# nanoporetech/bonito

Hardware: AMD Instinct MI355X
Metric: signal samples/sec/GPU (chunk=10000, batch=512) + read accuracy vs ref (higher is better)
Workload: dtype f16

## Files before the change

bonito_amd/csrc/conv.hip:

```cpp
#include "common.h"
#include "kernels.h"
#include "options.h"
#include <cstring>

namespace bh {

struct ConvFirstArgs {
    const half_t* sig;
    const float* w;
    const float* bias;
    half_t* out;
    int N, Lin, Lout, Cout, K, stride, pad, act;
    float clamp_lo, clamp_hi;
    long os_n, os_t;
    int vec8;
};

__global__ __launch_bounds__(256) void conv_first_kernel(ConvFirstArgs p) {
    extern __shared__ __attribute__((aligned(16))) char smem[];
    float* wl = (float*)smem;
    float* bl = wl + p.Cout * p.K;
    float* sl = bl + p.Cout;
    const int n = blockIdx.y;
    const int tb = blockIdx.x * 256;
    const int span = 255 * p.stride + p.K;
    const half_t* s = p.sig + (long)n * p.Lin;
    for (int i = threadIdx.x; i < p.Cout * p.K; i += 256) wl[i] = p.w[i];
    for (int i = threadIdx.x; i < p.Cout; i += 256) bl[i] = p.bias ? p.bias[i] : 0.0f;
    for (int i = threadIdx.x; i < span; i += 256) {
        int pos = tb * p.stride - p.pad + i;
        sl[i] = (pos >= 0 && pos < p.Lin) ? (float)s[pos] : 0.0f;
    }
    __syncthreads();
    const int t = tb + threadIdx.x;
    if (t >= p.Lout) return;
    const float* x = sl + threadIdx.x * p.stride;
    half_t* dst = p.out + (long)n * p.os_n + (long)t * p.os_t;
    auto channel = [&](int c) {
        const float* wr = wl + c * p.K;
        float a = bl[c];
        for (int k = 0; k < p.K; ++k) a = fmaf(wr[k], x[k], a);
        a = apply_act_rt(a, p.act);
        return (half_t)fminf(fmaxf(a, p.clamp_lo), p.clamp_hi);
    };
    int c0 = 0;
    if (p.vec8) {
        if (p.K == 5 && p.act == ACT_SWISH) {
            const float x0 = x[0], x1 = x[1], x2 = x[2], x3 = x[3], x4 = x[4];
            for (; c0 + 8 <= p.Cout; c0 += 8) {
                half8_t o;
#pragma unroll
                for (int j = 0; j < 8; ++j) {
                    const float* wr = wl + (c0 + j) * 5;
                    float a = bl[c0 + j];
                    a = fmaf(wr[0], x0, a);
                    a = fmaf(wr[1], x1, a);
                    a = fmaf(wr[2], x2, a);
                    a = fmaf(wr[3], x3, a);
                    a = fmaf(wr[4], x4, a);
                    o[j] = (half_t)fminf(fmaxf(swishf_(a), p.clamp_lo), p.clamp_hi);
                }
                *(half8_t*)(dst + c0) = o;
            }
        }
        for (; c0 + 8 <= p.Cout; c0 += 8) {
            half8_t o;
#pragma unroll
            for (int j = 0; j < 8; ++j) o[j] = channel(c0 + j);
            *(half8_t*)(dst + c0) = o;
        }
    }
    for (; c0 < p.Cout; ++c0) dst[c0] = channel(c0);
}

struct ConvArgs {
    const half_t* in;
    const half_t* wpk;
    const float* bias;
    half_t* out;
    int N, Lin, Lout, Cin, Cout, K, stride, pad, act;
    int Kp;
    float clamp_lo, clamp_hi;
    long os_n, os_t;
};

template <int NTT, bool FS = false>
__global__ __launch_bounds__(256) void conv_igemm_kernel(ConvArgs p) {
    extern __shared__ __attribute__((aligned(16))) char smem[];
    half_t* xin = (half_t*)smem;
    constexpr int PW = NTT * 16;
    constexpr int PB = 4 * PW;
    const int tid = threadIdx.x, lane = tid & 63, wave = tid >> 6;
    const int r = lane & 15, kg = lane >> 4;
    const int n = blockIdx.y;
    const int t0 = blockIdx.x * PB;

    const int span_pos = (PB - 1) * p.stride + p.K;
    const int span_halves = span_pos * p.Cin + 32 + 8;
    const int p_start = t0 * p.stride - p.pad;
    const half_t* src = p.in + (long)n * p.Lin * p.Cin;
    for (int e = tid * 8; e < span_halves; e += 256 * 8) {
        int pos = p_start + e / p.Cin;
        uint4_t v = {0, 0, 0, 0};
        if (pos >= 0 && pos < p.Lin && e < span_pos * p.Cin)
            v = *(const uint4_t*)(src + (long)pos * p.Cin + (e % p.Cin));
        *(uint4_t*)(xin + e) = v;
    }
    __syncthreads();

    const int nks = p.Kp >> 5;
    const int nft = (p.Cout + 15) >> 4;
    constexpr int NT = FS ? 4 * NTT : NTT;
    const int pbase = FS ? 0 : wave * PW;
    int boff[NT];
#pragma unroll
    for (int tt = 0; tt < NT; ++tt)
        boff[tt] = (pbase + tt * 16 + r) * p.stride * p.Cin + kg * 8;

    for (int ft = FS ? wave : 0; ft < nft; ft += FS ? 4 : 1) {
        float4_t acc[NT];
#pragma unroll
        for (int tt = 0; tt < NT; ++tt) acc[tt] = float4_t{0.f, 0.f, 0.f, 0.f};
        const half_t* wrow = p.wpk + (long)(ft * 16 + r) * p.Kp + kg * 8;
        int ks = 0;
        for (; FS && ks + 4 <= nks; ks += 4) {
            half8_t a[4];
#pragma unroll
            for (int u = 0; u < 4; ++u) a[u] = *(const half8_t*)(wrow + (ks + u) * 32);
#pragma unroll
            for (int u = 0; u < 4; ++u)
#pragma unroll
                for (int tt = 0; tt < NT; ++tt) {
                    half8_t b = *(const half8_t*)(xin + boff[tt] + (ks + u) * 32);
                    acc[tt] = mfma16(a[u], b, acc[tt]);
                }
        }
        for (; ks < nks; ++ks) {
            half8_t a = *(const half8_t*)(wrow + ks * 32);
#pragma unroll
            for (int tt = 0; tt < NT; ++tt) {
                half8_t b = *(const half8_t*)(xin + boff[tt] + ks * 32);
                acc[tt] = mfma16(a, b, acc[tt]);
            }
        }
        const int f = ft * 16 + kg * 4;
        if (f < p.Cout) {
            float bv[4];
#pragma unroll
            for (int g = 0; g < 4; ++g) bv[g] = (p.bias && f + g < p.Cout) ? p.bias[f + g] : 0.0f;
#pragma unroll
            for (int tt = 0; tt < NT; ++tt) {
                int t = t0 + pbase + tt * 16 + r;
                if (t >= p.Lout) continue;
                float xv[4];
#pragma unroll
                for (int g = 0; g < 4; ++g) xv[g] = acc[tt][g] + bv[g];
                if (p.act == ACT_SWISH) {
#pragma unroll
                    for (int g = 0; g < 4; ++g) xv[g] = swishf_(xv[g]);
                } else {
#pragma unroll
                    for (int g = 0; g < 4; ++g) xv[g] = apply_act_rt(xv[g], p.act);
                }
                half4_t o;
#pragma unroll
                for (int g = 0; g < 4; ++g) o[g] = (half_t)fminf(fmaxf(xv[g], p.clamp_lo), p.clamp_hi);
                half_t* dst = p.out + (long)n * p.os_n + (long)t * p.os_t + f;
                if (f + 4 <= p.Cout) *(half4_t*)dst = o;
                else
                    for (int g = 0; g < 4; ++g)
                        if (f + g < p.Cout) dst[g] = o[g];
            }
        }
    }
}

template <int FPW, int NKS, int WAVES>
__global__ __launch_bounds__(64 * WAVES) void conv_ws_kernel(ConvArgs p) {
    extern __shared__ __attribute__((aligned(16))) char smem[];
    half_t* xin = (half_t*)smem;
    constexpr int PB = 256;
    const int tid = threadIdx.x, lane = tid & 63, wave = tid >> 6;
    const int r = lane & 15, kg = lane >> 4;
    const int n = blockIdx.y;
    const int t0 = blockIdx.x * PB;

    half8_t afr[FPW][NKS];
#pragma unroll
    for (int f = 0; f < FPW; ++f) {
        const half_t* wrow = p.wpk + (long)((wave * FPW + f) * 16 + r) * p.Kp + kg * 8;
#pragma unroll
        for (int ks = 0; ks < NKS; ++ks) afr[f][ks] = *(const half8_t*)(wrow + ks * 32);
    }
    float4_t bv[FPW];
#pragma unroll
    for (int f = 0; f < FPW; ++f) {
        bv[f] = float4_t{0.f, 0.f, 0.f, 0.f};
        if (p.bias) bv[f] = *(const float4_t*)(p.bias + (wave * FPW + f) * 16 + kg * 4);
    }

    const int span_pos = (PB - 1) * p.stride + p.K;
    const int span_halves = span_pos * p.Cin + 32 + 8;
    const int p_start = t0 * p.stride - p.pad;
    const half_t* src = p.in + (long)n * p.Lin * p.Cin;
    for (int e = tid * 8; e < span_halves; e += 64 * WAVES * 8) {
        int pos = p_start + e / p.Cin;
        uint4_t v = {0, 0, 0, 0};
        if (pos >= 0 && pos < p.Lin && e < span_pos * p.Cin)
            v = *(const uint4_t*)(src + (long)pos * p.Cin + (e % p.Cin));
        *(uint4_t*)(xin + e) = v;
    }
    __syncthreads();

    const int RS = p.stride * p.Cin;
    for (int pt = 0; pt < PB / 16; ++pt) {
        const int t = t0 + pt * 16 + r;
        if (t0 + pt * 16 >= p.Lout) break;
        const half_t* xrow = xin + (pt * 16 + r) * RS + kg * 8;
        half8_t b[NKS];
#pragma unroll
        for (int ks = 0; ks < NKS; ++ks) b[ks] = *(const half8_t*)(xrow + ks * 32);
        float4_t acc[FPW];
#pragma unroll
        for (int f = 0; f < FPW; ++f) acc[f] = float4_t{0.f, 0.f, 0.f, 0.f};
#pragma unroll
        for (int ks = 0; ks < NKS; ++ks)
#pragma unroll
            for (int f = 0; f < FPW; ++f) acc[f] = mfma16(afr[f][ks], b[ks], acc[f]);
#pragma unroll
        for (int f = 0; f < FPW; ++f)
#pragma unroll
            for (int g = 0; g < 4; ++g) acc[f][g] += bv[f][g];
        switch (p.act) {
            case ACT_SWISH:
#pragma unroll
                for (int f = 0; f < FPW; ++f)
#pragma unroll
                    for (int g = 0; g < 4; ++g) acc[f][g] = swishf_(acc[f][g]);
                break;
            case ACT_TANH:
#pragma unroll
                for (int f = 0; f < FPW; ++f)
#pragma unroll
                    for (int g = 0; g < 4; ++g) acc[f][g] = tanhf_(acc[f][g]);
                break;
            case ACT_RELU:
#pragma unroll
                for (int f = 0; f < FPW; ++f)
#pragma unroll
                    for (int g = 0; g < 4; ++g) acc[f][g] = fmaxf(acc[f][g], 0.0f);
                break;
            default: break;
        }
        if (t < p.Lout) {
            half_t* drow = p.out + (long)n * p.os_n + (long)t * p.os_t + kg * 4;
#pragma unroll
            for (int f = 0; f < FPW; ++f) {
                half4_t o;
#pragma unroll
                for (int g = 0; g < 4; ++g) o[g] = (half_t)fminf(fmaxf(acc[f][g], p.clamp_lo), p.clamp_hi);
                *(half4_t*)(drow + (wave * FPW + f) * 16) = o;
            }
        }
    }
}

struct ConvFront3Args {
    const half_t* sig;
    const float* w1;
    const float* b1;
    const half_t* w2pk;
    const float* b2;
    int L0, L1, L2;
    int K1, pad1, act1;
    int K2, pad2, act2;
    float lo1, hi1, lo2, hi2;
    ConvArgs c3;
};

template <int FPW, int NKS, int WAVES>
__global__ __launch_bounds__(64 * WAVES) void conv_front3_kernel(ConvFront3Args q) {
    extern __shared__ __attribute__((aligned(16))) char smem[];
    const ConvArgs& p = q.c3;
    constexpr int PB = 256, CH = 256, C16 = 16, NT = 64 * WAVES;
    const int tid = threadIdx.x, lane = tid & 63, wave = tid >> 6;
    const int r = lane & 15, kg = lane >> 4;
    const int n = blockIdx.y;
    const int t0 = blockIdx.x * PB;
    const int span_pos = (PB - 1) * p.stride + p.K;
    const int span_halves = span_pos * C16 + 32 + 8;
    half_t* xin = (half_t*)smem;
    half_t* a1 = xin + ((span_halves + 7) & ~7);
    const int a1_rows = CH + q.K2 - 1 + 6;
    float* sl = (float*)(a1 + a1_rows * C16);
    float* wl = sl + span_pos + q.K2 - 1 + q.K1 - 1 + 8;
    float* bl = wl + C16 * q.K1;

    const int kp2 = ((q.K2 * 16 + 31) >> 5) << 5;
    half8_t a2[3];
#pragma unroll
    for (int ks = 0; ks < 3; ++ks) {
        a2[ks] = half8_t{0, 0, 0, 0, 0, 0, 0, 0};
        if (ks * 32 < kp2) a2[ks] = *(const half8_t*)(q.w2pk + (long)r * kp2 + kg * 8 + ks * 32);
    }
    float b2v[4];
#pragma unroll
    for (int g = 0; g < 4; ++g) b2v[g] = q.b2 ? q.b2[kg * 4 + g] : 0.0f;

    const int p3_start = t0 * p.stride - p.pad;
    const int s_start = p3_start - q.pad2 - q.pad1;
    const int s_len = span_pos + q.K2 - 1 + q.K1 - 1;
    const half_t* sg = q.sig + (long)n * q.L0;
    for (int i = tid; i < s_len; i += NT) {
        const int pos = s_start + i;
        sl[i] = (pos >= 0 && pos < q.L0) ? (float)sg[pos] : 0.0f;
    }
    for (int i = tid; i < C16 * q.K1; i += NT) wl[i] = q.w1[i];
    if (tid < C16) bl[tid] = q.b1 ? q.b1[tid] : 0.0f;
    for (int e = span_pos * C16 + tid; e < span_halves; e += NT) xin[e] = (half_t)0.0f;
    for (int e = (CH + q.K2 - 1) * C16 + tid; e < a1_rows * C16; e += NT) a1[e] = (half_t)0.0f;
    __syncthreads();
    const int c0t = (tid & 1) * 8;
    float w1r[8][5], w1b[8];
    if (q.K1 == 5) {
#pragma unroll
        for (int c = 0; c < 8; ++c) {
            w1b[c] = bl[c0t + c];
#pragma unroll
            for (int k = 0; k < 5; ++k) w1r[c][k] = wl[(c0t + c) * 5 + k];
        }
    }

    for (int q0 = 0; q0 < span_pos; q0 += CH) {
        const int rows1 = min(CH, span_pos - q0) + q.K2 - 1;
        if (q.K1 == 5) {
            for (int w = tid; w < 2 * rows1; w += NT) {
                const int i = w >> 1;
                const int u = p3_start + q0 - q.pad2 + i;
                const float* x = sl + (q0 + i);
                const float x0 = x[0], x1 = x[1], x2 = x[2], x3 = x[3], x4 = x[4];
                float av[8];
#pragma unroll
                for (int c = 0; c < 8; ++c) {
                    float a = w1b[c];
                    a = fmaf(w1r[c][0], x0, a);
                    a = fmaf(w1r[c][1], x1, a);
                    a = fmaf(w1r[c][2], x2, a);
                    a = fmaf(w1r[c][3], x3, a);
                    a = fmaf(w1r[c][4], x4, a);
                    av[c] = a;
                }
                if (q.act1 == ACT_SWISH) {
#pragma unroll
                    for (int c = 0; c < 8; ++c) av[c] = swishf_(av[c]);
                } else {
#pragma unroll
                    for (int c = 0; c < 8; ++c) av[c] = apply_act_rt(av[c], q.act1);
                }
                const bool inside = u >= 0 && u < q.L1;
                half8_t o;
#pragma unroll
                for (int c = 0; c < 8; ++c) o[c] = inside ? (half_t)fminf(fmaxf(av[c], q.lo1), q.hi1) : (half_t)0.0f;
                *(half8_t*)(a1 + i * C16 + c0t) = o;
            }
        } else
        for (int w = tid; w < 2 * rows1; w += NT) {
            const int i = w >> 1, c0 = (w & 1) * 8;
            const int u = p3_start + q0 - q.pad2 + i;
            const float* x = sl + (q0 + i);
            half8_t o;
#pragma unroll
            for (int c = 0; c < 8; ++c) {
                const float* wr = wl + (c0 + c) * q.K1;
                float a = bl[c0 + c];
                for (int k = 0; k < q.K1; ++k) a = fmaf(wr[k], x[k], a);
                a = apply_act_rt(a, q.act1);
                const half_t hv = (half_t)fminf(fmaxf(a, q.lo1), q.hi1);
                o[c] = (u >= 0 && u < q.L1) ? hv : (half_t)0.0f;
            }
            *(half8_t*)(a1 + i * C16 + c0) = o;
        }
        __syncthreads();
        const int tiles = (min(CH, span_pos - q0) + 15) >> 4;
        for (int pt = wave; pt < tiles; pt += WAVES) {
            const half_t* xrow = a1 + (pt * 16 + r) * C16 + kg * 8;
            float4_t acc = {0.f, 0.f, 0.f, 0.f};
#pragma unroll
            for (int ks = 0; ks < 3; ++ks) acc = mfma16(a2[ks], *(const half8_t*)(xrow + ks * 32), acc);
            const int j = q0 + pt * 16 + r;
            const int v = p3_start + j;
            float xv[4];
#pragma unroll
            for (int g = 0; g < 4; ++g) xv[g] = acc[g] + b2v[g];
            if (q.act2 == ACT_SWISH) {
#pragma unroll
                for (int g = 0; g < 4; ++g) xv[g] = swishf_(xv[g]);
            } else {
#pragma unroll
                for (int g = 0; g < 4; ++g) xv[g] = apply_act_rt(xv[g], q.act2);
            }
            const bool inside = v >= 0 && v < q.L2;
            half4_t o;
#pragma unroll
            for (int g = 0; g < 4; ++g) o[g] = inside ? (half_t)fminf(fmaxf(xv[g], q.lo2), q.hi2) : (half_t)0.0f;
            if (j < span_pos) *(half4_t*)(xin + j * C16 + kg * 4) = o;
        }
        __syncthreads();
    }

    half8_t afr[FPW][NKS];
#pragma unroll
    for (int f = 0; f < FPW; ++f) {
        const half_t* wrow = p.wpk + (long)((wave * FPW + f) * 16 + r) * p.Kp + kg * 8;
#pragma unroll
        for (int ks = 0; ks < NKS; ++ks) afr[f][ks] = *(const half8_t*)(wrow + ks * 32);
    }
    float4_t bv[FPW];
#pragma unroll
    for (int f = 0; f < FPW; ++f) {
        bv[f] = float4_t{0.f, 0.f, 0.f, 0.f};
        if (p.bias) bv[f] = *(const float4_t*)(p.bias + (wave * FPW + f) * 16 + kg * 4);
    }
    const int RS = p.stride * C16;
    for (int pt = 0; pt < PB / 16; ++pt) {
        const int t = t0 + pt * 16 + r;
        if (t0 + pt * 16 >= p.Lout) break;
        const half_t* xrow = xin + (pt * 16 + r) * RS + kg * 8;
        half8_t b[NKS];
#pragma unroll
        for (int ks = 0; ks < NKS; ++ks) b[ks] = *(const half8_t*)(xrow + ks * 32);
        float4_t acc[FPW];
#pragma unroll
        for (int f = 0; f < FPW; ++f) acc[f] = float4_t{0.f, 0.f, 0.f, 0.f};
#pragma unroll
        for (int ks = 0; ks < NKS; ++ks)
#pragma unroll
            for (int f = 0; f < FPW; ++f) acc[f] = mfma16(afr[f][ks], b[ks], acc[f]);
#pragma unroll
        for (int f = 0; f < FPW; ++f)
#pragma unroll
            for (int g = 0; g < 4; ++g) acc[f][g] += bv[f][g];
        switch (p.act) {
            case ACT_SWISH:
#pragma unroll
                for (int f = 0; f < FPW; ++f)
#pragma unroll
                    for (int g = 0; g < 4; ++g) acc[f][g] = swishf_(acc[f][g]);
                break;
            case ACT_TANH:
#pragma unroll
                for (int f = 0; f < FPW; ++f)
#pragma unroll
                    for (int g = 0; g < 4; ++g) acc[f][g] = tanhf_(acc[f][g]);
                break;
            case ACT_RELU:
#pragma unroll
                for (int f = 0; f < FPW; ++f)
#pragma unroll
                    for (int g = 0; g < 4; ++g) acc[f][g] = fmaxf(acc[f][g], 0.0f);
                break;
            default: break;
        }
        if (t < p.Lout) {
            half_t* drow = p.out + (long)n * p.os_n + (long)t * p.os_t + kg * 4;
#pragma unroll
            for (int f = 0; f < FPW; ++f) {
                half4_t o;
#pragma unroll
                for (int g = 0; g < 4; ++g) o[g] = (half_t)fminf(fmaxf(acc[f][g], p.clamp_lo), p.clamp_hi);
#ifdef BH_CONV_EXPT_NOSTORE
                if (o[0] == (half_t)12345.0f)
#endif
                *(half4_t*)(drow + (wave * FPW + f) * 16) = o;
            }
        }
    }
}

}

static int g_conv_last_kernel = 0;
void bh_k_conv_note_kernel(int code) { g_conv_last_kernel = code; }
int bh_k_conv_last_kernel() { return g_conv_last_kernel; }

int bh_k_conv_first(const void* signal, const float* w, const float* bias, void* out, int N, int Lin,
                    int Lout, int Cout, int K, int stride, int pad, int act, float clamp_lo,
                    float clamp_hi, long os_n, long os_t, hipStream_t stream) {
    using namespace bh;
    BH_REQUIRE(K >= 1 && Cout >= 1, "conv_first: bad shape (K=%d Cout=%d)", K, Cout);
    const int vec8 = (Cout % 8 == 0 && os_t % 8 == 0 && os_n % 8 == 0 && ((uintptr_t)out & 15) == 0) ? 1 : 0;
    ConvFirstArgs a{(const half_t*)signal, w, bias, (half_t*)out, N, Lin, Lout, Cout, K, stride, pad,
                    act, clamp_lo, clamp_hi, os_n, os_t, vec8};
    size_t lds = (size_t)(Cout * K + Cout + 255 * stride + K) * sizeof(float);
    hipLaunchKernelGGL(conv_first_kernel, dim3((Lout + 255) / 256, N), dim3(256), lds, stream, a);
    BH_CHECK_HIP(hipGetLastError());
    g_conv_last_kernel = BH_CONV_K_FIRST;
    return 0;
}

int bh_k_conv_igemm(const void* in, const void* wpk, const float* bias, void* out, int N, int Lin,
                    int Lout, int Cin, int Cout, int K, int stride, int pad, int act, float clamp_lo,
                    float clamp_hi, long os_n, long os_t, hipStream_t stream) {
    using namespace bh;
    BH_REQUIRE(Cin % 8 == 0 && Cout % 4 == 0, "conv_igemm: need Cin%%8==0, Cout%%4==0 (Cin=%d Cout=%d)", Cin, Cout);
    BH_REQUIRE(os_t % 4 == 0 && os_n % 4 == 0, "conv_igemm: output strides must be multiples of 4");
    ConvArgs a{(const half_t*)in, (const half_t*)wpk, bias, (half_t*)out, N, Lin, Lout, Cin, Cout, K,
               stride, pad, act, ((K * Cin + 31) / 32) * 32, clamp_lo, clamp_hi, os_n, os_t};
    auto lds_for = [&](int pw) { return (size_t)(((4 * pw - 1) * stride + K) * Cin + 40) * 2 + 16; };
    if (bh::g_opt.conv_ws && (Cout == 384 || Cout == 96) && a.Kp == 320 && lds_for(64) <= 64 * 1024 && ((uintptr_t)bias & 15) == 0) {
        const dim3 wgrid((Lout + 255) / 256, N);
        if (Cout == 384) hipLaunchKernelGGL((conv_ws_kernel<3, 10, 8>), wgrid, dim3(512), lds_for(64), stream, a);
        else hipLaunchKernelGGL((conv_ws_kernel<1, 10, 6>), wgrid, dim3(384), lds_for(64), stream, a);
        BH_CHECK_HIP(hipGetLastError());
        g_conv_last_kernel = Cout == 384 ? BH_CONV_K_WS_384 : BH_CONV_K_WS_96;
        return 0;
    }
    int pw = 64;
    while (pw > 16 && lds_for(pw) > (size_t)bh::g_opt.conv_lds_kb * 1024) pw >>= 1;
    size_t lds = lds_for(pw);
    BH_REQUIRE(lds <= 160 * 1024, "conv_igemm: input span does not fit LDS (%zu bytes)", lds);
    dim3 grid((Lout + 4 * pw - 1) / (4 * pw), N);
    if (lds > 64 * 1024) {
        const void* fn = pw == 64 ? (const void*)conv_igemm_kernel<4>
                         : pw == 32 ? (const void*)conv_igemm_kernel<2> : (const void*)conv_igemm_kernel<1>;
        BH_CHECK_HIP(bh_max_lds(fn, (int)lds));
    }
    const bool fs = bh::g_opt.conv_fs && Cout % 64 == 0;
    if (fs) {
        if (lds > 64 * 1024) {
            const void* fn = pw == 64 ? (const void*)conv_igemm_kernel<4, true>
                             : pw == 32 ? (const void*)conv_igemm_kernel<2, true> : (const void*)conv_igemm_kernel<1, true>;
            BH_CHECK_HIP(bh_max_lds(fn, (int)lds));
        }
        if (pw == 64) hipLaunchKernelGGL((conv_igemm_kernel<4, true>), grid, dim3(256), lds, stream, a);
        else if (pw == 32) hipLaunchKernelGGL((conv_igemm_kernel<2, true>), grid, dim3(256), lds, stream, a);
        else hipLaunchKernelGGL((conv_igemm_kernel<1, true>), grid, dim3(256), lds, stream, a);
    } else if (pw == 64) hipLaunchKernelGGL(conv_igemm_kernel<4>, grid, dim3(256), lds, stream, a);
    else if (pw == 32) hipLaunchKernelGGL(conv_igemm_kernel<2>, grid, dim3(256), lds, stream, a);
    else hipLaunchKernelGGL(conv_igemm_kernel<1>, grid, dim3(256), lds, stream, a);
    BH_CHECK_HIP(hipGetLastError());
    g_conv_last_kernel = BH_CONV_K_IGEMM(pw / 16, fs ? 1 : 0);
    return 0;
}


static size_t conv_front3_lds(int K1, int K2, int K3, int s3) {
    const size_t span = (size_t)255 * s3 + K3;
    return ((span * 16 + 40 + 7) & ~(size_t)7) * 2 + (size_t)(256 + K2 - 1 + 6) * 16 * 2 + (span + K2 + K1 + 6) * 4 + (size_t)(16 * K1 + 16) * 4;
}
static int conv_front3_kp(int K3) { return ((K3 * 16 + 31) / 32) * 32; }
int bh_k_conv_front3_shape_ok(int K1, int K2, int c3_out, int K3, int s3) {
    if (K1 < 1 || K1 > 8 || K2 < 1 || K2 * 16 > 96 || K3 < 1 || s3 < 1) return 0;
    if (!(c3_out == 384 || c3_out == 96) || conv_front3_kp(K3) != 320) return 0;
    return conv_front3_lds(K1, K2, K3, s3) <= 80 * 1024 ? 1 : 0;
}
int bh_k_conv_front3_option_ok(int c3_out) {
    if (!bh::g_opt.conv_fuse || !bh::g_opt.conv_ws) return 0;
    return (c3_out == 96 && bh::g_opt.conv_fuse < 2) ? 0 : 1;
}
int bh_k_conv_front3_ok(int c1_eff, int K1, int s1, int c2_in_eff, int c2_eff, int K2, int s2, int c3_in_eff, int c3_out, int K3, int s3) {
    if (c1_eff != 16 || c2_in_eff != 16 || c2_eff != 16 || c3_in_eff != 16 || s1 != 1 || s2 != 1) return 0;
    return bh_k_conv_front3_shape_ok(K1, K2, c3_out, K3, s3) && bh_k_conv_front3_option_ok(c3_out);
}

int bh_k_conv_front3(const void* signal, int N, int L0, const float* w1, const float* b1, int K1, int pad1, int act1, float lo1, float hi1,
                     const void* w2pk, const float* b2, int K2, int pad2, int act2, float lo2, float hi2, const void* w3pk,
                     const float* b3, int Cout3, int K3, int stride3, int pad3, int act3, float lo3, float hi3, void* out, long os_n,
                     long os_t, hipStream_t stream) {
    using namespace bh;
    BH_REQUIRE(bh_k_conv_front3_shape_ok(K1, K2, Cout3, K3, stride3),
               "conv_front3: no instance for K1=%d K2=%d Cout3=%d K3=%d stride3=%d (bh_k_conv_front3_shape_ok)", K1, K2, Cout3, K3, stride3);
    BH_REQUIRE(((uintptr_t)b3 & 15) == 0, "conv_front3: conv3's bias must be 16-byte aligned (or null)");
    const int L1 = L0 + 2 * pad1 - K1 + 1, L2 = L1 + 2 * pad2 - K2 + 1, L3 = (L2 + 2 * pad3 - K3) / stride3 + 1;
    BH_REQUIRE(L1 > 0 && L2 > 0 && L3 > 0, "conv_front3: chunk of %d samples is too short", L0);
    BH_REQUIRE(os_t % 4 == 0 && os_n % 4 == 0, "conv_front3: output strides must be multiples of 4");
    ConvFront3Args a{(const half_t*)signal, w1, b1, (const half_t*)w2pk, b2, L0, L1, L2, K1, pad1, act1, K2, pad2, act2, lo1, hi1, lo2, hi2,
                     ConvArgs{nullptr, (const half_t*)w3pk, b3, (half_t*)out, N, L2, L3, 16, Cout3, K3, stride3, pad3, act3, conv_front3_kp(K3), lo3, hi3,
                              os_n, os_t}};
    const size_t lds = conv_front3_lds(K1, K2, K3, stride3);
    const dim3 grid((L3 + 255) / 256, N);
    if (Cout3 == 384) {
        if (lds > 64 * 1024) BH_CHECK_HIP(bh_max_lds((const void*)conv_front3_kernel<3, 10, 8>, (int)lds));
        hipLaunchKernelGGL((conv_front3_kernel<3, 10, 8>), grid, dim3(512), lds, stream, a);
    } else {
        if (lds > 64 * 1024) BH_CHECK_HIP(bh_max_lds((const void*)conv_front3_kernel<1, 10, 6>, (int)lds));
        hipLaunchKernelGGL((conv_front3_kernel<1, 10, 6>), grid, dim3(384), lds, stream, a);
    }
    BH_CHECK_HIP(hipGetLastError());
    g_conv_last_kernel = Cout3 == 384 ? BH_CONV_K_FRONT3_384 : BH_CONV_K_FRONT3_96;
    return 0;
}
```

bonito_amd/csrc/options.cpp:

```cpp
#include "options.h"

#include <string.h>

namespace bh {

Options g_opt;

#define BH_OPT(name) #name, &Options::name
static constexpr OptionRow OPTION_TABLE[] = {
    {BH_OPT(gemm_path), 0, Norm::keep, "linear GEMM kernel families: 0 auto, 1 = v1 only, 2 = no 256-tile kernel, 3 = no four-wave kernel, 5 = four-wave wherever legal"},
    {BH_OPT(gemm_tile16), 1, Norm::flag, "four-wave GEMM K-tile stream: 1 = 16x16x32 MFMAs, 0 = 32x32x16 (agree to fp16 rounding)"},
    {BH_OPT(gemm_order), 1, Norm::flag, "four-wave GEMM work order in an XCD: 1 = feature groups fastest, 0 = token blocks fastest (same bytes)"},
    {BH_OPT(gemm_gf), 0, Norm::keep, "four-wave GEMM feature tiles per block: 0 automatic, else rounded down to 1 / 2 / 4 / 8 / 16 / 32 (same bytes)"},
    {BH_OPT(gemm_stagger), 0, Norm::keep, "start-phase stagger of the persistent GEMM kernels, 0 = off (same bytes; measured without effect)"},
    {BH_OPT(attn_waves), 0, Norm::keep, "ring attention waves per workgroup: 0 automatic, 8, 12 (same results)"},
    {BH_OPT(attn_version), 2, Norm::one_or_two, "ring attention kernel: 2 = current, 1 = the first ring kernel"},
    {BH_OPT(attn_expt), 0, Norm::keep, "timing experiments of the ring attention kernel (bit mask): RESULTS ARE WRONG ON PURPOSE unless 0"},
    {BH_OPT(beam_fork), -1, Norm::keep, "posterior scan next to the beam kernel on a helper stream: -1 auto, 0 never, 1 always"},
    {BH_OPT(beam_select), 0, Norm::keep, "beam top-W selection: 0 histogram + boundary ranking, 1 radix search (same beams)"},
    {BH_OPT(beam_fuse), -1, Norm::keep, "forward / posterior scan as a second wave of the beam kernel: -1 auto (<= 256 states), 0 never, 1 always"},
    {BH_OPT(beam_cpw), 0, Norm::keep, "chunks per workgroup of the fused beam kernel at 256 states: 0 automatic, 1, 2, 4 (same bytes)"},
    {BH_OPT(decode_nt), 0, Norm::keep, "non-temporal score loads in the decode scans: 0 off"},
    {BH_OPT(viterbi_quad), 1, Norm::keep, "CRF Viterbi: 1 = four states per thread where the layout allows, 0 = the one-state kernel everywhere"},
    {BH_OPT(conv_ws), 1, Norm::keep, "weight-stationary kernel for the 384- / 96-channel 19-tap convolution: 1 on, 0 = generic implicit GEMM"},
    {BH_OPT(conv_fs), 1, Norm::keep, "feature-split instances of the implicit-GEMM convolution: 1 on, 0 = position-split"},
    {BH_OPT(conv_fuse), 1, Norm::keep, "conv1 -> conv2 -> conv3 as one kernel: 1 = 384-channel stacks, 2 = also 96-channel, 0 = three kernels"},
    {BH_OPT(conv_lds_kb), 64, Norm::positive_or_def, "KiB of LDS a workgroup of the implicit-GEMM convolution may take for its input span"},
    {BH_OPT(lstm_max_spins), 1000000, Norm::nonneg_or_def, "bound of the recurrent kernels' exchange spin loops (0: the first incomplete poll round is a timeout)"},
    {BH_OPT(lstm_q8_variant), 0, Norm::keep, "geometry of the 8-bit recurrent kernel, read at bh_encoder_create: 0, 1, 2"},
};
#undef BH_OPT

static constexpr bool defaults_agree() {
    constexpr Options o{};
    for (const OptionRow& r : OPTION_TABLE)
        if (o.*r.member != r.def) return false;
    return true;
}
static_assert(defaults_agree(), "options.h and OPTION_TABLE state different defaults");
static_assert(sizeof(OPTION_TABLE) / sizeof(OPTION_TABLE[0]) == sizeof(Options) / sizeof(int), "every member of Options has exactly one row");

const OptionRow* find_option(const char* name) {
    for (const OptionRow& r : OPTION_TABLE)
        if (!strcmp(name, r.name)) return &r;
    return nullptr;
}

}
```

bonito_amd/csrc/options.h:

```cpp
#pragma once

namespace bh {

struct Options {
    int gemm_path = 0;
    int gemm_tile16 = 1;
    int gemm_order = 1;
    int gemm_gf = 0;
    int gemm_stagger = 0;
    int attn_waves = 0;
    int attn_version = 2;
    int attn_expt = 0;
    int beam_fork = -1;
    int beam_select = 0;
    int beam_fuse = -1;
    int beam_cpw = 0;
    int decode_nt = 0;
    int viterbi_quad = 1;
    int conv_ws = 1;
    int conv_fs = 1;
    int conv_fuse = 1;
    int conv_lds_kb = 64;
    int lstm_max_spins = 1000000;
    int lstm_q8_variant = 0;
};
extern Options g_opt;

enum class Norm {
    keep,
    flag,
    one_or_two,
    positive_or_def,
    nonneg_or_def
};
struct OptionRow {
    const char* name;
    int Options::*member;
    int def;
    Norm norm;
    const char* what;
    int normalise(int v) const {
        switch (norm) {
            case Norm::flag: return v ? 1 : 0;
            case Norm::one_or_two: return v == 1 ? 1 : 2;
            case Norm::positive_or_def: return v > 0 ? v : def;
            case Norm::nonneg_or_def: return v >= 0 ? v : def;
            default: return v;
        }
    }
};
const OptionRow* find_option(const char* name);

}
```

Baseline: 409.8 million.

## Pipeline fused conv front end with producer waves computing next block's conv1/conv2

Adds a persistent 12-wave kernel for the 384-channel fused conv1->conv2->conv3 front end. Four producer waves run at raised priority and compute conv1 and conv2 for the next 256-position block into a double-buffered LDS span, while eight consumer waves run the conv3 MFMA GEMM on the current block. The grid is one workgroup per CU, each walking a contiguous range of work items. This is meant to overlap the serial front-end phases and remove per-block launch and weight reload costs, at the price of more LDS and a block-wide barrier per iteration.

```diff
diff --git a/bonito_amd/csrc/conv.hip b/bonito_amd/csrc/conv.hip
--- a/bonito_amd/csrc/conv.hip
+++ b/bonito_amd/csrc/conv.hip
@@ -477,6 +477,264 @@
     }
 }
 
+static __device__ __forceinline__ float clamp_med3(float x, float lo, float hi) { return __builtin_amdgcn_fmed3f(x, lo, hi); }
+
+static __device__ __forceinline__ void wave_lds_sync() {
+    __builtin_amdgcn_fence(__ATOMIC_RELEASE, "wavefront");
+    __builtin_amdgcn_wave_barrier();
+    __builtin_amdgcn_fence(__ATOMIC_ACQUIRE, "wavefront");
+}
+
+constexpr int PIPE_CW = 8, PIPE_PW = 4, PIPE_SL = 64;
+constexpr int PIPE_A1R = PIPE_SL + 5 + 7;
+constexpr int PIPE_NSV = (PIPE_SL + 12 + 63) / 64;
+constexpr int PIPE_SG = PIPE_SL + 5 + 7 + 4;
+
+template <int FPW, int NKS>
+__global__ __launch_bounds__(64 * (PIPE_CW + PIPE_PW)) void conv_front3_pipe_kernel(ConvFront3Args q, int nb, int total) {
+    extern __shared__ __attribute__((aligned(16))) char smem[];
+    const ConvArgs& p = q.c3;
+    constexpr int PB = 256, C16 = 16, NT = 64 * (PIPE_CW + PIPE_PW);
+    const int tid = threadIdx.x, lane = tid & 63;
+    const int wave = __builtin_amdgcn_readfirstlane(tid >> 6);
+    const int r = lane & 15, kg = lane >> 4;
+    const int span_pos = (PB - 1) * p.stride + p.K;
+    const int span_halves = span_pos * C16 + 32 + 8;
+    const int xin_halves = (span_halves + 7) & ~7;
+    half_t* xin0 = (half_t*)smem;
+    half_t* a1all = xin0 + 2 * xin_halves;
+    float* slall = (float*)(a1all + PIPE_PW * PIPE_A1R * C16);
+    float* wl = slall + PIPE_PW * PIPE_SG;
+    float* bl = wl + C16 * q.K1;
+    float* b3l = bl + C16;
+
+    const int first = (int)((long)blockIdx.x * total / gridDim.x);
+    const int nrun = (int)((long)(blockIdx.x + 1) * total / gridDim.x) - first;
+
+    for (int i = tid; i < C16 * q.K1; i += NT) wl[i] = q.w1[i];
+    if (tid < C16) bl[tid] = q.b1 ? q.b1[tid] : 0.0f;
+    for (int i = tid; i < C16 * FPW * PIPE_CW; i += NT) b3l[i] = p.bias ? p.bias[i] : 0.0f;
+    for (int b = 0; b < 2; ++b)
+        for (int e = span_pos * C16 + tid; e < span_halves; e += NT) xin0[b * xin_halves + e] = (half_t)0.0f;
+    for (int e = tid; e < PIPE_PW * PIPE_A1R * C16; e += NT) a1all[e] = (half_t)0.0f;
+    __syncthreads();
+
+    if (wave >= PIPE_CW) {
+        __builtin_amdgcn_s_setprio(1);
+        const int pw = wave - PIPE_CW;
+        half_t* a1 = a1all + pw * PIPE_A1R * C16;
+        float* sl = slall + pw * PIPE_SG;
+        const int kp2 = ((q.K2 * 16 + 31) >> 5) << 5;
+        half8_t a2[3];
+#pragma unroll
+        for (int ks = 0; ks < 3; ++ks) {
+            a2[ks] = half8_t{0, 0, 0, 0, 0, 0, 0, 0};
+            if (ks * 32 < kp2) a2[ks] = *(const half8_t*)(q.w2pk + (long)r * kp2 + kg * 8 + ks * 32);
+        }
+        float b2v[4];
+#pragma unroll
+        for (int g = 0; g < 4; ++g) b2v[g] = q.b2 ? q.b2[kg * 4 + g] : 0.0f;
+        const int c0t = (lane & 1) * 8;
+        float w1r[8][5], w1b[8];
+        if (q.K1 == 5) {
+#pragma unroll
+            for (int c = 0; c < 8; ++c) {
+                w1b[c] = bl[c0t + c];
+#pragma unroll
+                for (int k = 0; k < 5; ++k) w1r[c][k] = wl[(c0t + c) * 5 + k];
+            }
+        }
+        const int halo = q.K2 - 1;
+        half_t sv[PIPE_NSV];
+        auto fetch = [&](const half_t* sg, int s0, int len) {
+#pragma unroll
+            for (int u = 0; u < PIPE_NSV; ++u) {
+                const int i = lane + 64 * u, pos = s0 + i;
+                sv[u] = (half_t)0.0f;
+                if (i < len && pos >= 0 && pos < q.L0) sv[u] = sg[pos];
+            }
+        };
+        __builtin_amdgcn_s_waitcnt(0x0F70);
+        for (int it = 0; it <= nrun; ++it) {
+            if (it < nrun) {
+                const int item = first + it, n = item / nb, t0 = (item - n * nb) * PB;
+                half_t* xin = xin0 + (it & 1) * xin_halves;
+                const int p3_start = t0 * p.stride - p.pad;
+                const int vt = min(PB, (p.Lout - t0 + 15) & ~15);
+                const int rows = min(span_pos, (vt - 1) * p.stride + 2 * NKS);
+                const int ntl = (rows + 15) >> 4;
+                const int tlo = ntl * pw / PIPE_PW, thi = ntl * (pw + 1) / PIPE_PW;
+                const half_t* sg = q.sig + (long)n * q.L0;
+                for (int ts = tlo; ts < thi; ts += PIPE_SL / 16) {
+                    const int nt = min(PIPE_SL / 16, thi - ts);
+                    const int r0 = ts * 16;
+                    const int u0 = p3_start + r0 - q.pad2, s0 = u0 - q.pad1;
+                    const bool head = ts == tlo;
+                    wave_lds_sync();
+                    if (head) fetch(sg, s0, nt * 16 + halo + q.K1 - 1);
+#pragma unroll
+                    for (int u = 0; u < PIPE_NSV; ++u)
+                        if (lane + 64 * u < nt * 16 + halo + q.K1 - 1) sl[lane + 64 * u] = (float)sv[u];
+                    if (ts + PIPE_SL / 16 < thi) fetch(sg, s0 + PIPE_SL, min(PIPE_SL / 16, thi - ts - PIPE_SL / 16) * 16 + halo + q.K1 - 1);
+                    if (!head && lane < 2 * halo)
+                        *(half8_t*)(a1 + lane * 8) = *(const half8_t*)(a1 + PIPE_SL * C16 + lane * 8);
+                    wave_lds_sync();
+                    const int i_lo = head ? 0 : halo, i_hi = nt * 16 + halo;
+                    if (q.K1 == 5) {
+                        for (int w = 2 * i_lo + lane; w < 2 * i_hi; w += 64) {
+                            const int i = w >> 1;
+                            const int u = u0 + i;
+                            const float* x = sl + i;
+                            const float x0 = x[0], x1 = x[1], x2 = x[2], x3 = x[3], x4 = x[4];
+                            float av[8];
+#pragma unroll
+                            for (int c = 0; c < 8; ++c) {
+                                float a = w1b[c];
+                                a = fmaf(w1r[c][0], x0, a);
+                                a = fmaf(w1r[c][1], x1, a);
+                                a = fmaf(w1r[c][2], x2, a);
+                                a = fmaf(w1r[c][3], x3, a);
+                                a = fmaf(w1r[c][4], x4, a);
+                                av[c] = a;
+                            }
+                            if (q.act1 == ACT_SWISH) {
+#pragma unroll
+                                for (int c = 0; c < 8; ++c) av[c] = swishf_(av[c]);
+                            } else {
+#pragma unroll
+                                for (int c = 0; c < 8; ++c) av[c] = apply_act_rt(av[c], q.act1);
+                            }
+                            const bool inside = u >= 0 && u < q.L1;
+                            half8_t o;
+#pragma unroll
+                            for (int c = 0; c < 8; ++c) o[c] = inside ? (half_t)clamp_med3(av[c], q.lo1, q.hi1) : (half_t)0.0f;
+                            *(half8_t*)(a1 + i * C16 + c0t) = o;
+                        }
+                    } else
+                    for (int w = 2 * i_lo + lane; w < 2 * i_hi; w += 64) {
+                        const int i = w >> 1;
+                        const int u = u0 + i;
+                        const float* x = sl + i;
+                        half8_t o;
+#pragma unroll
+                        for (int c = 0; c < 8; ++c) {
+                            const float* wr = wl + (c0t + c) * q.K1;
+                            float a = bl[c0t + c];
+                            for (int k = 0; k < q.K1; ++k) a = fmaf(wr[k], x[k], a);
+                            a = apply_act_rt(a, q.act1);
+                            const half_t hv = (half_t)fminf(fmaxf(a, q.lo1), q.hi1);
+                            o[c] = (u >= 0 && u < q.L1) ? hv : (half_t)0.0f;
+                        }
+                        *(half8_t*)(a1 + i * C16 + c0t) = o;
+                    }
+                    wave_lds_sync();
+#pragma unroll
+                    for (int tt = 0; tt < PIPE_SL / 16; ++tt) {
+                        if (tt < nt) {
+                            const half_t* xrow = a1 + (tt * 16 + r) * C16 + kg * 8;
+                            float4_t acc = {0.f, 0.f, 0.f, 0.f};
+#pragma unroll
+                            for (int ks = 0; ks < 3; ++ks) acc = mfma16(a2[ks], *(const half8_t*)(xrow + ks * 32), acc);
+                            const int j = r0 + tt * 16 + r;
+                            const int v = p3_start + j;
+                            float xv[4];
+#pragma unroll
+                            for (int g = 0; g < 4; ++g) xv[g] = acc[g] + b2v[g];
+                            if (q.act2 == ACT_SWISH) {
+#pragma unroll
+                                for (int g = 0; g < 4; ++g) xv[g] = swishf_(xv[g]);
+                            } else {
+#pragma unroll
+                                for (int g = 0; g < 4; ++g) xv[g] = apply_act_rt(xv[g], q.act2);
+                            }
+                            const bool inside = v >= 0 && v < q.L2;
+                            half4_t o;
+#pragma unroll
+                            for (int g = 0; g < 4; ++g) o[g] = inside ? (half_t)clamp_med3(xv[g], q.lo2, q.hi2) : (half_t)0.0f;
+                            if (j < span_pos) *(half4_t*)(xin + j * C16 + kg * 4) = o;
+                        }
+                    }
+                }
+            }
+            __syncthreads();
+        }
+    } else {
+        half8_t afr[FPW][NKS];
+#pragma unroll
+        for (int f = 0; f < FPW; ++f) {
+            const half_t* wrow = p.wpk + (long)((wave * FPW + f) * 16 + r) * p.Kp + kg * 8;
+#pragma unroll
+            for (int ks = 0; ks < NKS; ++ks) afr[f][ks] = *(const half8_t*)(wrow + ks * 32);
+        }
+        const int RS = p.stride * C16;
+        __builtin_amdgcn_s_waitcnt(0x0F70);
+        for (int it = 0; it <= nrun; ++it) {
+            if (it >= 1) {
+                const int item = first + it - 1, n = item / nb, t0 = (item - n * nb) * PB;
+                const half_t* xin = xin0 + ((it - 1) & 1) * xin_halves;
+                int ln;
+                asm volatile("v_mbcnt_lo_u32_b32 %0, -1, 0\n\tv_mbcnt_hi_u32_b32 %0, -1, %0" : "=v"(ln));
+                const int r = ln & 15, kg = ln >> 4;
+                for (int pt = 0; pt < PB / 16; ++pt) {
+                    const int t = t0 + pt * 16 + r;
+                    if (t0 + pt * 16 >= p.Lout) break;
+                    const half_t* xrow = xin + (pt * 16 + r) * RS + kg * 8;
+                    half8_t b[NKS];
+#pragma unroll
+                    for (int ks = 0; ks < NKS; ++ks) b[ks] = *(const half8_t*)(xrow + ks * 32);
+                    float4_t acc[FPW];
+#pragma unroll
+                    for (int f = 0; f < FPW; ++f) acc[f] = float4_t{0.f, 0.f, 0.f, 0.f};
+#pragma unroll
+                    for (int ks = 0; ks < NKS; ++ks)
+#pragma unroll
+                        for (int f = 0; f < FPW; ++f) acc[f] = mfma16(afr[f][ks], b[ks], acc[f]);
+                    int bo = (wave * FPW * 16 + kg * 4) * 4;
+                    asm volatile("" : "+v"(bo));
+#pragma unroll
+                    for (int f = 0; f < FPW; ++f) {
+                        const float4_t bv = *(const float4_t*)((const char*)b3l + bo + f * 64);
+#pragma unroll
+                        for (int g = 0; g < 4; ++g) acc[f][g] += bv[g];
+                    }
+                    switch (p.act) {
+                        case ACT_SWISH:
+#pragma unroll
+                            for (int f = 0; f < FPW; ++f)
+#pragma unroll
+                                for (int g = 0; g < 4; ++g) acc[f][g] = swishf_(acc[f][g]);
+                            break;
+                        case ACT_TANH:
+#pragma unroll
+                            for (int f = 0; f < FPW; ++f)
+#pragma unroll
+                                for (int g = 0; g < 4; ++g) acc[f][g] = tanhf_(acc[f][g]);
+                            break;
+                        case ACT_RELU:
+#pragma unroll
+                            for (int f = 0; f < FPW; ++f)
+#pragma unroll
+                                for (int g = 0; g < 4; ++g) acc[f][g] = fmaxf(acc[f][g], 0.0f);
+                            break;
+                        default: break;
+                    }
+                    if (t < p.Lout) {
+                        half_t* drow = p.out + (long)n * p.os_n + (long)t * p.os_t + kg * 4;
+#pragma unroll
+                        for (int f = 0; f < FPW; ++f) {
+                            half4_t o;
+#pragma unroll
+                            for (int g = 0; g < 4; ++g) o[g] = (half_t)clamp_med3(acc[f][g], p.clamp_lo, p.clamp_hi);
+                            *(half4_t*)(drow + (wave * FPW + f) * 16) = o;
+                        }
+                    }
+                }
+            }
+            __syncthreads();
+        }
+    }
+}
+
 }
 
 static int g_conv_last_kernel = 0;
@@ -549,6 +807,10 @@
     return ((span * 16 + 40 + 7) & ~(size_t)7) * 2 + (size_t)(256 + K2 - 1 + 6) * 16 * 2 + (span + K2 + K1 + 6) * 4 + (size_t)(16 * K1 + 16) * 4;
 }
 static int conv_front3_kp(int K3) { return ((K3 * 16 + 31) / 32) * 32; }
+static size_t conv_front3_pipe_lds(int K1, int K3, int s3) {
+    const size_t span = (size_t)255 * s3 + K3;
+    return 2 * ((span * 16 + 40 + 7) & ~(size_t)7) * 2 + (size_t)bh::PIPE_PW * bh::PIPE_A1R * 16 * 2 + (size_t)bh::PIPE_PW * bh::PIPE_SG * 4 + (size_t)(16 * K1 + 16 + 384) * 4;
+}
 int bh_k_conv_front3_shape_ok(int K1, int K2, int c3_out, int K3, int s3) {
     if (K1 < 1 || K1 > 8 || K2 < 1 || K2 * 16 > 96 || K3 < 1 || s3 < 1) return 0;
     if (!(c3_out == 384 || c3_out == 96) || conv_front3_kp(K3) != 320) return 0;
@@ -577,6 +839,20 @@
     ConvFront3Args a{(const half_t*)signal, w1, b1, (const half_t*)w2pk, b2, L0, L1, L2, K1, pad1, act1, K2, pad2, act2, lo1, hi1, lo2, hi2,
                      ConvArgs{nullptr, (const half_t*)w3pk, b3, (half_t*)out, N, L2, L3, 16, Cout3, K3, stride3, pad3, act3, conv_front3_kp(K3), lo3, hi3,
                               os_n, os_t}};
+    if (Cout3 == 384 && bh::g_opt.conv_front_pipe) {
+        const size_t plds = conv_front3_pipe_lds(K1, K3, stride3);
+        const int nb = (L3 + 255) / 256;
+        const long total = (long)N * nb;
+        BH_REQUIRE(total < (1l << 30), "conv_front3: %ld blocks are more than the pipelined kernel indexes", total);
+        long wgs = bh_cu_count() > 0 ? bh_cu_count() : 256;
+        if (bh::g_opt.conv_front_wgs > 0 && bh::g_opt.conv_front_wgs < wgs) wgs = bh::g_opt.conv_front_wgs;
+        if (wgs > total) wgs = total;
+        BH_CHECK_HIP(bh_max_lds((const void*)conv_front3_pipe_kernel<3, 10>, (int)plds));
+        hipLaunchKernelGGL((conv_front3_pipe_kernel<3, 10>), dim3((unsigned)wgs), dim3(64 * (PIPE_CW + PIPE_PW)), plds, stream, a, nb, (int)total);
+        BH_CHECK_HIP(hipGetLastError());
+        g_conv_last_kernel = BH_CONV_K_FRONT3_384;
+        return 0;
+    }
     const size_t lds = conv_front3_lds(K1, K2, K3, stride3);
     const dim3 grid((L3 + 255) / 256, N);
     if (Cout3 == 384) {
diff --git a/bonito_amd/csrc/options.cpp b/bonito_amd/csrc/options.cpp
--- a/bonito_amd/csrc/options.cpp
+++ b/bonito_amd/csrc/options.cpp
@@ -26,6 +26,8 @@
     {BH_OPT(conv_fs), 1, Norm::keep, "feature-split instances of the implicit-GEMM convolution: 1 on, 0 = position-split"},
     {BH_OPT(conv_fuse), 1, Norm::keep, "conv1 -> conv2 -> conv3 as one kernel: 1 = 384-channel stacks, 2 = also 96-channel, 0 = three kernels"},
     {BH_OPT(conv_lds_kb), 64, Norm::positive_or_def, "KiB of LDS a workgroup of the implicit-GEMM convolution may take for its input span"},
+    {BH_OPT(conv_front_pipe), 1, Norm::keep, "fused front end of the 384-channel stacks: 1 = conv1 / conv2 of the next block beside conv3 (12-wave pipeline), 0 = phase after phase (same bytes)"},
+    {BH_OPT(conv_front_wgs), 0, Norm::keep, "workgroups of the pipelined front end: 0 = one per CU, n > 0 caps the grid (same bytes; test hook, A/B)"},
     {BH_OPT(lstm_max_spins), 1000000, Norm::nonneg_or_def, "bound of the recurrent kernels' exchange spin loops (0: the first incomplete poll round is a timeout)"},
     {BH_OPT(lstm_q8_variant), 0, Norm::keep, "geometry of the 8-bit recurrent kernel, read at bh_encoder_create: 0, 1, 2"},
 };
diff --git a/bonito_amd/csrc/options.h b/bonito_amd/csrc/options.h
--- a/bonito_amd/csrc/options.h
+++ b/bonito_amd/csrc/options.h
@@ -21,6 +21,8 @@
     int conv_fs = 1;
     int conv_fuse = 1;
     int conv_lds_kb = 64;
+    int conv_front_pipe = 1;
+    int conv_front_wgs = 0;
     int lstm_max_spins = 1000000;
     int lstm_q8_variant = 0;
 };
```

Result: faster. 431.5 million, median of 6 (+5.3%).
